# hhcho/sfgwas

Hardware: AMD Instinct MI355X
Metric: pca_power_iter_ring_macs_per_s (higher is better)
Workload: dtype u64 ring words, exact integers: int8 digits on the matrix core for the MAC of all five moduli, fp64-held integers in the encode and key-switch kernels

## Files before the change

sfgwas_amd/csrc/kernels.hpp:

```cpp
#pragma once
#include "common.hpp"
#include "mm_plan.hpp"
#include "assoc_plan.hpp"

constexpr int SFG_MAXPATTERN = 128;
struct ModPattern { int period; int8_t m[SFG_MAXPATTERN]; };
struct RowMap { int rpg; size_t gstride_in, gstride_out; };
struct PanelMap { int G, g, shift0; unsigned packed_mask = 0; int K = 0; };

int launch_ntt_fwd(sfg_ctx *ctx, const u64 *in, u64 *out, size_t nrows, const ModPattern &pat);
int launch_ntt_inv(sfg_ctx *ctx, const u64 *in, u64 *out, size_t nrows, const ModPattern &pat);
int launch_ntt_plain(sfg_ctx *ctx, const double *pc, u64 *out, size_t nplain, int L);
struct MoveJob;
struct PtRide;
int launch_ntt_plain_half(sfg_ctx *ctx, const double *pc, u64 *out_half, size_t nplain, int L, PanelMap pm, const uint32_t *perm = nullptr, const MoveJob *mv = nullptr);
int launch_expand_half(sfg_ctx *ctx, const u64 *half, u64 *full, size_t nrows);
int launch_ntt_fwd_map(sfg_ctx *ctx, const u64 *in, u64 *out, size_t nrows, const ModPattern &pat, const RowMap &rm);
int launch_ntt_inv_map(sfg_ctx *ctx, const u64 *in, u64 *out, size_t nrows, const ModPattern &pat, const RowMap &rm);
struct MacStrides { size_t rot_k, rot_r, pt_k, pt_n, out_n, out_r; bool pt_half = false; bool pt_packed = false; bool pt_digits = false; bool i8 = false; bool i8_big = false; bool pt_digits_big = false;
                    const int8_t *B_small = nullptr, *B_big = nullptr;
                    int pt_layout = 0, pt_L = 0;
                    int B_mode = 0;
                    const int8_t *A_small = nullptr, *A_big = nullptr; };
int launch_mac_i8_small(sfg_ctx *ctx, const double *rotf, size_t rotf_k_stride, size_t rotf_r_stride, int plane0, const u64 *pt, u64 *out, int K, int R, int r0, int Ncols,
                        int l0, int nl, int accumulate, const MacStrides &st);
int launch_mac_i8_big(sfg_ctx *ctx, const double *rotf, size_t rotf_k_stride, size_t rotf_r_stride, int plane0, const u64 *pt, u64 *out, int K, int R, int r0, int Ncols,
                      int l0, int accumulate, const MacStrides &st);
int launch_skew(sfg_ctx *ctx, const int8_t *blk, size_t ld, int r, int c, int transposed, int square, int8_t *D);
struct PcCache { double *slot = nullptr; int mode = 0; const uint32_t *perm = nullptr; };
int launch_encode_rows(sfg_ctx *ctx, const int8_t *D, int shift0, int nshift, int L, u64 *pt, bool half_rows = false, int G = 0, int g = 0, unsigned packed_mask = 0, const PcCache *pcache = nullptr,
                       PtRide *ride = nullptr);
int encode_rows_launches(const sfg_ctx *ctx, int nshift);
int i8_ride_prepare(sfg_ctx *ctx, const u64 *panel, int K, int Ncols, size_t pt_k, size_t pt_n, int layout, int L, int launches, PtRide &ride);
int i8_ride_finish(sfg_ctx *ctx, PtRide &ride);
int i8_ride_tiles(sfg_ctx *ctx, int K, int L, int8_t **Bs, int8_t **Bb);
struct I8Args;
void launch_i8_pack_pt_digits(hipStream_t q, const I8Args &a, unsigned items, bool big);
void launch_move_alone(hipStream_t q, const MoveJob &j);
int launch_share(sfg_ctx *ctx, const u64 *rows, size_t rows_ct_stride, const u64 *xr, size_t x_ct_stride, u64 *h, int nl, int nct);
int launch_add_rows(sfg_ctx *ctx, const u64 *a, size_t a_ct_stride, const u64 *b, size_t b_ct_stride, u64 *out, size_t out_ct_stride, int nl, int nct);
int encrypt_errors_moddown(sfg_ctx *ctx, const int32_t *e0, const int32_t *e1, int nct, int level, u64 *out);
int launch_geno_unpack(sfg_ctx *ctx, const sfg_geno *g, size_t r0, size_t c0, size_t nr, size_t nc, int8_t *out, size_t ld_out);
int launch_rotate_right(sfg_ctx *ctx, const u64 *in, u64 *out, int nct, int level, const int *nrot_host);
int launch_rotate_right_indexed(sfg_ctx *ctx, const u64 *in, int nin, u64 *out, int nct, int level, const int *nrot_host, const int *in_index);
int launch_rotate_right_indexed_f64(sfg_ctx *ctx, const u64 *in, int nin, double *outf, int nct, int level, const int *nrot_host, const int *in_index, int L,
                                    const size_t *out_slot = nullptr);
int launch_relinearize(sfg_ctx *ctx, const u64 *tmp, int nct, int level, const u64 *mid, u64 *out);
int launch_ct_add(sfg_ctx *ctx, const u64 *a, const u64 *b, u64 *out, size_t nct, int level);
int mac_dma_planes(sfg_ctx *ctx, int L, std::vector<int> &plane_of, std::vector<int> &is_big);
double mac_big_maxterm(u64 q);
int launch_rot_to_f64(sfg_ctx *ctx, const u64 *rot, size_t nrows, int nl_rot, int L, double *rotf);
int launch_mac_dma(sfg_ctx *ctx, const double *rotf, size_t rows_per_k, const u64 *pt, u64 *out, int K, int R, int Ncols, int L, int accumulate, const MacStrides &st,
                   const double *rotsum = nullptr);
int launch_rot_sum(sfg_ctx *ctx, const double *rotf, size_t rows_per_k, int K, int L, double *rotsum);
int launch_pack_pt(sfg_ctx *ctx, const u64 *in, u64 *out, size_t nrows, size_t words_per_row, int L, unsigned packed_mask);
unsigned mac_dma_packed_mask(sfg_ctx *ctx, int L);
bool mac_use_dma(const sfg_ctx *ctx);
int launch_mac_bc(sfg_ctx *ctx, const double *rotf, size_t rows_per_k, const u64 *pt, u64 *out, int K, int R, int Ncols, int L, int accumulate, const MacStrides &st,
                  const double *rotsum);
int rotcache_build_rows_tab(sfg_ctx *ctx, const u64 *A, int s, int in_level, int max_level, int nbr, int b0, int b1, const std::vector<std::vector<uint8_t>> *tabs, double *cache);
int assoc_build_rotcache(sfg_ctx *ctx, const u64 *A_dev, int s, int in_level, int max_level, size_t nr, const std::vector<size_t> &widths, double **out);
struct I8RotPre { int G = 0, nbr = 0, s = 0, L = 0; std::vector<int8_t *> As, Ab; };
int i8_rotpre_build(sfg_ctx *ctx, const u64 *A_dev, int s, int in_level, int max_level, int nbr, const std::vector<std::vector<uint8_t>> *tabs, size_t budget_bytes, const char *prefix, I8RotPre &pre);
void i8_rotpre_free(I8RotPre &pre);
int matmul_resident_range_i8pre(sfg_ctx *ctx, const I8RotPre &pre, int s, int max_level, const sfg_geno *g, unsigned flags, int blk0, int blk1, uint64_t *out);
int matmul_accumulate_i8pre(sfg_ctx *ctx, const I8RotPre &pre, int s, int max_level, const sfg_geno *g, unsigned flags, int j0, int j1, int accumulate, uint64_t *acc,
                            size_t acc_col_words = 0);
int launch_i8_pack_rot_to(sfg_ctx *ctx, const double *rotf, size_t rotf_k_stride, size_t rotf_r_stride, int plane0, int K, int R, int l0, int nl, bool big, int8_t *A_out);
struct AssocRot { double *f64 = nullptr; I8RotPre pre; };
int assoc_build_rot(sfg_ctx *ctx, const u64 *A_dev, int s, int in_level, int max_level, size_t nr, const std::vector<size_t> &widths, AssocRot &out);
void assoc_free_rot(AssocRot &r);
struct AssocRotScope { AssocRot r; ~AssocRotScope() { assoc_free_rot(r); } };
int assoc_product(sfg_ctx *ctx, const AssocRot &r, const uint64_t *A_dev, int s, int in_level, int max_level, const sfg_geno *g, unsigned flags, int nct, uint64_t *out);
int assoc_batch_tail(sfg_ctx *ctx, const u64 *tmp, const sfg_geno *g, int s, size_t nct, size_t ctw, uint64_t *out_dev, size_t out_ct_capacity, size_t out_shift,
                     double *sum_host, double *sqsum_host);

int launch_bed_decode(sfg_ctx *ctx, hipStream_t st, const uint8_t *dbed, size_t bps, size_t num_sample, size_t num_snp, const int32_t *rmap, const int32_t *cmap,
// ... 10 lines not shown
```

sfgwas_amd/csrc/matmul.hip:

```cpp
#include "common.hpp"
#include "kernels.hpp"
#include "i8_move.hpp"
#include <algorithm>
#include <string>

static inline int ceil_div(size_t a, size_t b) { return (int)((a + b - 1) / b); }

struct Shape {
    size_t nrow, ncol;
    int nbr, m_ct;
    bool transposed;
    const int8_t *dev; size_t ld;
    const sfg_geno *g;
    int rows_of(int bi) const { return (int)(std::min((size_t)(bi + 1) * SFG_SLOTS, nrow) - (size_t)bi * SFG_SLOTS); }
    int cols_of(int bj) const { return (int)(std::min((size_t)(bj + 1) * SFG_SLOTS, ncol) - (size_t)bj * SFG_SLOTS); }
    const int8_t *block(int bi, int bj) const {
        return transposed ? dev + (size_t)bj * SFG_SLOTS * ld + (size_t)bi * SFG_SLOTS
                          : dev + (size_t)bi * SFG_SLOTS * ld + (size_t)bj * SFG_SLOTS;
    }
};
static Shape make_shape(const sfg_geno *g, unsigned flags) {
    Shape sh; sh.transposed = (flags & SFG_TRANSPOSE) != 0;
    sh.nrow = sh.transposed ? g->ncol : g->nrow; sh.ncol = sh.transposed ? g->nrow : g->ncol;
    sh.nbr = ceil_div(sh.nrow, SFG_SLOTS); sh.m_ct = ceil_div(sh.ncol, SFG_SLOTS);
    sh.dev = g->dev; sh.ld = g->ld; sh.g = g; return sh;
}

__global__ void __launch_bounds__(256) k_drop_level(const u64 *in, u64 *out, int nl_in, int nl) {
    const int N = SFG_N; const size_t row = blockIdx.x / (N / 256);
    const size_t ctp = row / nl, m = row % nl;
    const size_t x = (blockIdx.x % (N / 256)) * 256 + threadIdx.x;
    out[row * N + x] = in[(ctp * nl_in + m) * N + x];
}
__global__ void __launch_bounds__(256) k_sum_giants(const u64 *rot, int ngiant, int s, int L, u64 *out, size_t out_i_stride,
                                                    int accumulate, const ModConst *modc) {
    const int N = SFG_N; const size_t row = blockIdx.x / (N / 256);
    const int i = (int)(row / (2 * L)), pl = (int)(row % (2 * L)), l = pl % L;
    const size_t x = (blockIdx.x % (N / 256)) * 256 + threadIdx.x;
    const double q = modc[l].q, qinv = modc[l].qinv;
    double acc = accumulate ? u64_to_f64(out[(size_t)i * out_i_stride + (size_t)pl * N + x]) : 0.0;
    for (int g = 0; g < ngiant; g++) {
        acc += u64_to_f64(rot[(((size_t)g * s + i) * 2 * L + pl) * N + x]);
        if ((g & 31) == 31) acc = pred(acc, q, qinv);
    }
    out[(size_t)i * out_i_stride + (size_t)pl * N + x] = f64_to_u64(canon(acc, q, qinv));
}
__global__ void __launch_bounds__(256) k_reduce_rows(u64 *rows, int L, const ModConst *modc) {
    const int N = SFG_N; const size_t row = blockIdx.x / (N / 256); const int l = (int)(row % L);
    const size_t off = row * N + (blockIdx.x % (N / 256)) * 256 + threadIdx.x;
    rows[off] = rows[off] % modc[l].qi;
}
__global__ void __launch_bounds__(256) k_pt_zero(u64 *pt, size_t pitch_words, size_t seg_words, int L, size_t prow, unsigned packed_mask) {
    const size_t seg = blockIdx.y, x = (size_t)blockIdx.x * 256 + threadIdx.x;
    if (x >= seg_words) return;
    const int l = (int)((x / prow) % L);
    pt[seg * pitch_words + x] = ((packed_mask >> l) & 1u) ? PACKED_ZERO : 0ULL;
}
__global__ void __launch_bounds__(256) k_pt_zero_kmajor(uint8_t *pt, int K, int planes, int n0, int k0, int nk) {
    const size_t blk = ((size_t)(n0 + blockIdx.y) * planes * 64 + blockIdx.x) * (size_t)K * 128 + (size_t)k0 * 128;
    uint4 *p = reinterpret_cast<uint4 *>(pt + blk);
    for (int i = threadIdx.x; i < nk * 8; i += 256) p[i] = make_uint4(0, 0, 0, 0);
}
static int launch_pt_zero_kmajor(sfg_ctx *ctx, u64 *pt, int K, int planes, int n0, int n1, int k0, int k1) {
    if (n1 <= n0 || k1 <= k0) return 0;
    hipLaunchKernelGGL(k_pt_zero_kmajor, dim3((unsigned)(planes * 64), (unsigned)(n1 - n0)), dim3(256), 0, ctx->stream, reinterpret_cast<uint8_t *>(pt), K, planes, n0, k0, k1 - k0);
    SFG_HIP(ctx, hipGetLastError());
    return 0;
}
static int launch_pt_zero(sfg_ctx *ctx, u64 *pt, size_t pitch_words, size_t seg_words, int nseg, int L, size_t prow, unsigned packed_mask) {
    if (!packed_mask) {
        if (nseg == 1) SFG_HIP(ctx, hipMemsetAsync(pt, 0, seg_words * 8, ctx->stream));
        else SFG_HIP(ctx, hipMemset2DAsync(pt, pitch_words * 8, 0, seg_words * 8, nseg, ctx->stream));
        return 0;
    }
    hipLaunchKernelGGL(k_pt_zero, dim3((unsigned)((seg_words + 255) / 256), (unsigned)nseg), dim3(256), 0, ctx->stream, pt, pitch_words, seg_words, L, prow, packed_mask);
    SFG_HIP(ctx, hipGetLastError());
    return 0;
}
// ... 452 lines not shown
                SFG_HIP(ctx, hipEventRecord(ctx->ev_pipe[(gi + 1) & 1], ctx->aux_stream));
            }
            SFG_HIP(ctx, hipStreamWaitEvent(main_stream, ctx->ev_pipe[gi & 1], 0));
            rotf_grp = c.rotf + (size_t)(gi & 1) * rot_half;
            if (c.rotsum) rotsum_grp = c.rotsum + (size_t)(gi & 1) * rotsum_half;
        } else SFG_TRY(build_group(c, bg, b1, 0));
        for (int bj = j0; bj < j1; bj++, it++) {
            pt = pt_base + (size_t)(plan.ride_want ? (it & 1) : 0) * plan.panel_words;
            PtRide ride;
            if (plan.ride_want && !c.rideBs) SFG_TRY(i8_ride_tiles(ctx, G * d, L, &c.rideBs, &c.rideBb));
            if (held.on && plan.ride_want && c.rideBs) {
                SFG_TRY(i8_ride_prepare(ctx, held.ptp, held.gsn * d, d, plan.plw, (size_t)held.gsn * d * plan.plw, plan.pt_layout, L, ride_launch_count(c, bg, ng, sh.cols_of(bj)), ride));
                if (ride.on && (ride.job.a5.B != c.rideBs || (ride.job.n6 && ride.job.a6.B != c.rideBb))) SFG_FAIL(ctx, "matmul: internal: the riding transposition's tile buffers moved");
            }
            if (held.on && !ride.on) { SFG_TRY(run_mac(c, held, c.rideBs ? 2 : 0)); held.on = false; }
            for (int g = 0; g < ng; g++) SFG_TRY(encode_block(c, bg + g, bj, g, ng, pt, ride.on ? &ride : nullptr));
            if (held.on) { SFG_TRY(i8_ride_finish(ctx, ride)); SFG_TRY(run_mac(c, held, 1)); held.on = false; }
            MacJob m; m.on = true; m.ptp = pt; m.gsn = ng; m.gi = gi;
            m.acc_flag = (accumulate || bg != b0) ? 1 : 0;
            m.accj = acc + (size_t)(bj - j0) * acc_col; m.rotf_grp = rotf_grp; m.rotsum_grp = rotsum_grp;
            if (plan.ride_want && c.rideBs) held = m;
            else SFG_TRY(run_mac(c, m, c.rideBs ? 2 : 0));
        }
    }
    if (held.on) rc = run_mac(c, held, 2);
    return rc;
}

static int matmul_finalize(sfg_ctx *ctx, const u64 *acc, int s, int max_level, int ncolb, int m_ct_out, int jout0, int g0, int g1,
                           const std::vector<uint8_t> *giant_active, int accumulate, u64 *out, int acc_giants = SFG_D, int giant_base = 0) {
    const int N = SFG_N, d = SFG_D, L = max_level;
    const size_t accw = (size_t)s * 2 * L * N, ctw = (size_t)2 * L * N;
    if (g0 < 0 || g1 > acc_giants || g0 > g1 || giant_base < 0) SFG_FAIL(ctx, "finalize: giant range out of bounds");
    u64 *rot = nullptr;
    SFG_TRY(sfg_scratch(ctx, "mm.fin_rot", (size_t)d * accw * 8, (void **)&rot));
    std::vector<int> glist;
    for (int g = g0; g < g1; g++) if (giant_base + g < d && (!giant_active || (*giant_active)[giant_base + g])) glist.push_back(g);
    const int ng = (int)glist.size();
    std::vector<int> nrv((size_t)ng * s), inv((size_t)ng * s);
    for (int k = 0; k < ng; k++) for (int i = 0; i < s; i++) { nrv[(size_t)k * s + i] = -(giant_base + glist[k]) * d; inv[(size_t)k * s + i] = glist[k] * s + i; }
    int rc = 0;
    for (int jb = 0; jb < ncolb && !rc; jb++) {
        const u64 *accj = acc + (size_t)jb * acc_giants * accw;
        u64 *o = out + (size_t)(jout0 + jb) * ctw;
        if (ng) {
            PhaseTimer t(ctx, "rotate");
            rc = launch_rotate_right_indexed(ctx, accj, acc_giants * s, rot, ng * s, L - 1, nrv.data(), inv.data());
            t.stop(1);
            if (rc) break;
        }
        hipLaunchKernelGGL(k_sum_giants, dim3((unsigned)((size_t)s * 2 * L * (N / 256))), dim3(256), 0, ctx->stream, rot, ng, s, L,
                           o, (size_t)m_ct_out * ctw, accumulate, ctx->modc);
        if (hipGetLastError() != hipSuccess) { rc = 1; ctx->err = "finalize: k_sum_giants launch failed"; }
    }
    return rc;
}

static void giant_table(const Shape &sh, std::vector<uint8_t> &giant_t) {
    giant_t.assign(SFG_D, 0);
    for (int bi = 0; bi < sh.nbr; bi++) {
        const int nr = sh.rows_of(bi);
        for (int shift = 0; shift < SFG_SLOTS; shift++) {
            if (giant_t[shift / SFG_D]) { shift = (shift / SFG_D + 1) * SFG_D - 1; continue; }
            bool any = false;
            for (int bj = 0; bj < sh.m_ct && !any; bj++) any = diag_bool(nr, sh.cols_of(bj), SFG_SLOTS, -shift);
            if (any) giant_t[shift / SFG_D] = 1;
        }
    }
}

extern "C" int sfg_matmul_accumulate_dev(sfg_ctx *ctx, const uint64_t *A, int s, int in_level, int max_level, const sfg_geno *g, unsigned flags,
                                         int b0, int b1, int j0, int j1, int accumulate, uint64_t *acc) {
    ApiScope api_scope(ctx);
    SFG_HIP(ctx, hipSetDevice(ctx->device));
    Shape sh = make_shape(g, flags);
    return matmul_accumulate(ctx, (const u64 *)A, s, in_level, max_level, sh, flags, b0, b1, j0, j1, accumulate, (u64 *)acc);
}
extern "C" int sfg_matmul_finalize_dev(sfg_ctx *ctx, const uint64_t *acc, int s, int max_level, int ncolb, int g0, int g1, int accumulate, uint64_t *out) {
    ApiScope api_scope(ctx);
    SFG_HIP(ctx, hipSetDevice(ctx->device));
    return matmul_finalize(ctx, (const u64 *)acc, s, max_level, ncolb, ncolb, 0, g0, g1, nullptr, accumulate, (u64 *)out);
}

extern "C" int sfg_matmul_finalize_slots_dev(sfg_ctx *ctx, const uint64_t *acc, int s, int max_level, int ncolb, int acc_giants, int giant_base,
                                             int g0, int g1, int accumulate, uint64_t *out) {
    ApiScope api_scope(ctx);
    SFG_HIP(ctx, hipSetDevice(ctx->device));
    if (acc_giants < 1) SFG_FAIL(ctx, "finalize: acc_giants must be positive");
// ... 515 lines not shown
```

sfgwas_amd/csrc/rotate.hip:

```cpp
#include "common.hpp"
#include "kernels.hpp"
#include "ksw.hpp"


static void fill_ext(const sfg_ctx *ctx, ExtConst &e, const std::vector<int> &src) {
    memset(&e, 0, sizeof e);
    e.a = (int)src.size();
    for (int m = 0; m < e.a; m++) e.src[m] = src[m];
    for (int m = 0; m < e.a; m++) {
        u64 qm = ctx->q[src[m]], h = 1;
        for (int k = 0; k < e.a; k++) if (k != m) h = h_mulmod(h, ctx->q[src[k]] % qm, qm);
        u64 hi = h_invmod(h, qm);
        e.qhat_inv[m] = (double)hi; e.qhat_inv_q[m] = (double)hi / (double)qm;
    }
    for (int t = 0; t < ctx->nmod; t++) {
        u64 qt = ctx->q[t], D = 1 % qt;
        for (int m = 0; m < e.a; m++) {
            u64 ht = 1 % qt;
            for (int k = 0; k < e.a; k++) if (k != m) ht = h_mulmod(ht, ctx->q[src[k]] % qt, qt);
            e.qhat_t[t][m] = (double)ht; e.qhat_t_q[t][m] = (double)ht / (double)qt;
            D = h_mulmod(D, ctx->q[src[m]] % qt, qt);
        }
        e.D_t[t] = (double)D; e.D_t_q[t] = (double)D / (double)qt;
    }
// ... 22 lines not shown
    }
    *host = kc;
    auto it = ctx->ksw_cache.find(level);
    if (it == ctx->ksw_cache.end()) {
        KswConst *d = nullptr;
        SFG_HIP(ctx, hipMalloc(&d, sizeof(KswConst)));
        SFG_HIP(ctx, hipMemcpy(d, &kc, sizeof(KswConst), hipMemcpyHostToDevice));
        ctx->ksw_cache[level] = d; *dev = d;
    } else *dev = (KswConst *)it->second;
    return 0;
}


__global__ void __launch_bounds__(256) k_ksw_extend(const u64 *c2, const u64 *ct_in, u64 *ext, const KswConst *kcp, const ModConst *modc) {
    const KswConst &kc = *kcp;
    const int N = SFG_N, x = blockIdx.x * 256 + threadIdx.x, i = blockIdx.y; const size_t b = blockIdx.z;
    const ExtConst &e = kc.dig[i];
    const u64 *c2b = c2 + b * (size_t)kc.nl * N;
    u64 *eb = ext + (b * kc.beta + i) * (size_t)kc.nt * N;
    double xs[KSW_MAXA], y[KSW_MAXA], v = 0.0;
#pragma unroll
    for (int m = 0; m < KSW_MAXA; m++) xs[m] = m < e.a ? u64_to_f64(c2b[(size_t)e.src[m] * N + x]) : 0.0;
    if (e.a > 1) ext_prepare(e, modc, xs, y, v);
    for (int t = 0; t < kc.nt; t++) {
        const int tg = kc.tmod[t];
        u64 outv;
        if (kc.digit_of[t] == i) continue;
        else if (e.a == 1) outv = f64_to_u64(canon(xs[0], modc[tg].q, modc[tg].qinv));
        else outv = f64_to_u64(ext_target(e, tg, modc[tg].q, modc[tg].qinv, y, v));
        eb[(size_t)t * N + x] = outv;
    }
}

__global__ void __launch_bounds__(256) k_ksw_inner(const u64 *ext, const u64 *ct_in, const u64 *const *keys, const int *inidx, u64 *acc, const KswConst *kcp, const ModConst *modc, int nmod) {
    const KswConst &kc = *kcp;
    const int N = SFG_N, x = 2 * (blockIdx.x * 256 + threadIdx.x), t = blockIdx.y; const size_t b = blockIdx.z;
    const int tg = kc.tmod[t];
    const double q = modc[tg].q, qinv = modc[tg].qinv;
    const u64 *key = keys[b];
    const size_t bi = (size_t)inidx[b];
    double a0x = 0.0, a0y = 0.0, a1x = 0.0, a1y = 0.0;
    for (int i = 0; i < kc.beta; i++) {
        const ulonglong2 ev = kc.digit_of[t] == i ? *reinterpret_cast<const ulonglong2 *>(ct_in + (bi * 2 * (size_t)kc.nl + kc.nl + t) * N + x)
                                                  : *reinterpret_cast<const ulonglong2 *>(ext + ((bi * kc.beta + i) * (size_t)kc.nt + t) * N + x);
        const ulonglong2 k0 = *reinterpret_cast<const ulonglong2 *>(key + (((size_t)i * 2 + 0) * nmod + tg) * N + x);
        const ulonglong2 k1 = *reinterpret_cast<const ulonglong2 *>(key + (((size_t)i * 2 + 1) * nmod + tg) * N + x);
        const double ex = u64_to_f64(ev.x), ey = u64_to_f64(ev.y);
        a0x += mulmod2(ex, u64_to_f64(k0.x), q, qinv); a0y += mulmod2(ey, u64_to_f64(k0.y), q, qinv);
        a1x += mulmod2(ex, u64_to_f64(k1.x), q, qinv); a1y += mulmod2(ey, u64_to_f64(k1.y), q, qinv);
    }
    *reinterpret_cast<ulonglong2 *>(acc + ((b * 2 + 0) * (size_t)kc.nt + t) * N + x) = make_ulonglong2(f64_to_u64(canon(a0x, q, qinv)), f64_to_u64(canon(a0y, q, qinv)));
    *reinterpret_cast<ulonglong2 *>(acc + ((b * 2 + 1) * (size_t)kc.nt + t) * N + x) = make_ulonglong2(f64_to_u64(canon(a1x, q, qinv)), f64_to_u64(canon(a1y, q, qinv)));
}

__global__ void __launch_bounds__(256) k_moddown_extend(const u64 *acc, u64 *ext2, const KswConst *kcp, const ModConst *modc) {
    const KswConst &kc = *kcp;
    const int N = SFG_N, x = blockIdx.x * 256 + threadIdx.x, p = blockIdx.y; const size_t b = blockIdx.z;
    const ExtConst &e = kc.pq;
    const u64 *ap = acc + ((b * 2 + p) * (size_t)kc.nt + kc.nl) * N;
    double xs[KSW_MAXA], y[KSW_MAXA], v = 0.0;
#pragma unroll
    for (int m = 0; m < KSW_MAXA; m++) xs[m] = m < e.a ? u64_to_f64(ap[(size_t)m * N + x]) : 0.0;
    if (e.a > 1) ext_prepare(e, modc, xs, y, v);
    for (int t = 0; t < kc.nl; t++) {
        u64 outv = e.a == 1 ? f64_to_u64(canon(xs[0], modc[t].q, modc[t].qinv)) : f64_to_u64(ext_target(e, t, modc[t].q, modc[t].qinv, y, v));
        ext2[((b * 2 + p) * (size_t)kc.nl + t) * N + x] = outv;
    }
}

struct F64Form { int on, L, centre; size_t rowf; int plane_of[SFG_MAXMOD], big[SFG_MAXMOD]; };
__device__ __forceinline__ void store_rot_f64(double *row, const F64Form &ff, int t, int x, double v, double q) {
    const int N = SFG_N;
    double *o = row + (size_t)ff.plane_of[t] * N;
    if (ff.big[t]) {
        const double wc = v > __builtin_floor(q * 0.5) ? v - q : v;
        const double hi = __builtin_floor((wc + 4194304.0) * 0x1p-23), lo = wc - hi * 8388608.0;
        o[2 * x] = lo; o[2 * x + 1] = hi;
    } else o[x] = (ff.centre && v > __builtin_floor(q * 0.5)) ? v - q : v;
}
__global__ void __launch_bounds__(256) k_ksw_finish(const u64 *ct_in, const int *inidx, const u64 *acc, const u64 *ext2, const uint16_t *const *index,
                                                   u64 *const *ct_out, const KswConst *kcp, const ModConst *modc, const u64 *add1, F64Form ff) {
    const KswConst &kc = *kcp;
    const int N = SFG_N, x = blockIdx.x * 256 + threadIdx.x, t = blockIdx.y; const size_t b = blockIdx.z;
    if (ff.on && t >= ff.L) return;
    const double q = modc[t].q, qinv = modc[t].qinv, pinv = kc.pinv[t], pinv_q = kc.pinv_q[t];
    const int src = index[b][x];
#pragma unroll
    for (int p = 0; p < 2; p++) {
        const double a = u64_to_f64(acc[((b * 2 + p) * (size_t)kc.nt + t) * N + src]);
        const double e = u64_to_f64(ext2[((b * 2 + p) * (size_t)kc.nl + t) * N + src]);
        double r = mulmod_lazy(a - e, pinv, pinv_q, q);
        if (p == 0) r += u64_to_f64(ct_in[((size_t)inidx[b] * 2 * (size_t)kc.nl + t) * N + src]);
        else if (add1) r += u64_to_f64(add1[((size_t)inidx[b] * (size_t)kc.nl + t) * N + src]);
        const double v = canon(r, q, qinv);
        if (ff.on) store_rot_f64(reinterpret_cast<double *>(ct_out[b]) + (size_t)p * ff.rowf, ff, t, x, v, q);
        else ct_out[b][((size_t)p * kc.nl + t) * N + x] = f64_to_u64(v);
    }
}

__global__ void __launch_bounds__(256) k_ct_add(const u64 *a, const u64 *b, u64 *out, int nl, const ModConst *modc, size_t total_rows) {
    const int N = SFG_N; const size_t row = blockIdx.x / (N / 256); const int m = (int)(row % nl);
    const u64 q = modc[m].qi;
    const size_t off = row * N + (blockIdx.x % (N / 256)) * 256 + threadIdx.x;
    u64 v = a[off] + b[off]; out[off] = v >= q ? v - q : v;
}

static int launch_keyswitch_jobs(sfg_ctx *ctx, const u64 *in, int nin, int level, const std::vector<int> &job_in, const std::vector<const u64 *> &keyp,
                                 const std::vector<const uint16_t *> &idxp, const std::vector<u64 *> &outp, const u64 *add1, const F64Form *ffp = nullptr) {
    const int N = SFG_N, nl = level + 1;
    F64Form ff; memset(&ff, 0, sizeof ff); if (ffp) ff = *ffp;
    KswConst *kcd; KswConst kc;
    SFG_TRY(get_ksw(ctx, level, &kcd, &kc));
    const size_t ctw = (size_t)2 * nl * N;
    const int nr = (int)job_in.size();
    if (!nr) return 0;
    const size_t in_rows = (size_t)nl + (size_t)kc.beta * kc.nt, job_rows = 2 * (size_t)kc.nt + 2 * (size_t)nl;
    const size_t budget = ctx->cfg.ksw_budget;
    int in_grp = (int)(budget / (in_rows * N * 8)); if (in_grp < 1) in_grp = 1; if (in_grp > nin) in_grp = nin;
    int chunk = (int)(budget / (job_rows * N * 8)); if (chunk < 1) chunk = 1; if (chunk > nr) chunk = nr;
    const size_t ptr_bytes = (size_t)nr * (3 * sizeof(void *) + sizeof(int)) + 256;
    const size_t ext_rows = (size_t)in_grp * kc.beta * kc.nt, ext2_rows = (size_t)chunk * 2 * nl;
    SFG_TRY(sfg_ws_reserve(ctx, (in_rows * in_grp + job_rows * chunk + ext_rows + ext2_rows) * N * 8 + ptr_bytes));
    u64 *c2 = (u64 *)ctx->ws, *ext = c2 + (size_t)in_grp * nl * N;
    u64 *acc = ext + ext_rows * N, *ext2 = acc + (size_t)chunk * 2 * kc.nt * N;
    u64 *extT = ext2 + ext2_rows * N, *ext2T = extT + ext_rows * N;
    const u64 **keys_all = (const u64 **)(ext2T + ext2_rows * N);
    const uint16_t **idx_all = (const uint16_t **)(keys_all + nr);
    u64 **out_all = (u64 **)(idx_all + nr);
    int *inidx_all = (int *)(out_all + nr);
    ModPattern pq; pq.period = nl; for (int m = 0; m < nl; m++) pq.m[m] = (int8_t)m;
    ModPattern pext; pext.period = kc.beta * kc.nt;
    for (int i = 0; i < kc.beta; i++) for (int t = 0; t < kc.nt; t++) pext.m[i * kc.nt + t] = kc.digit_of[t] == i ? (int8_t)-2 : (int8_t)kc.tmod[t];
    ModPattern pp; pp.period = kc.np; for (int p = 0; p < kc.np; p++) pp.m[p] = (int8_t)(ctx->nq + p);
    for (int i0 = 0; i0 < nin; i0 += in_grp) {
        const int ni = nin - i0 < in_grp ? nin - i0 : in_grp;
        std::vector<int> jobs;
        for (int k = 0; k < nr; k++) if (job_in[k] >= i0 && job_in[k] < i0 + ni) jobs.push_back(k);
        if (jobs.empty()) continue;
        const u64 *bin = in + (size_t)i0 * ctw;
        RowMap rm1; rm1.rpg = nl; rm1.gstride_in = ctw; rm1.gstride_out = (size_t)nl * N;
        SFG_TRY(launch_ntt_inv_map(ctx, bin + (size_t)nl * N, c2, (size_t)ni * nl, pq, rm1));
        hipLaunchKernelGGL(k_ksw_extend, dim3(N / 256, kc.beta, ni), dim3(256), 0, ctx->stream, c2, bin, ext, kcd, ctx->modc);
        SFG_HIP(ctx, hipGetLastError());
        SFG_TRY(launch_ntt_fwd(ctx, ext, extT, (size_t)ni * kc.beta * kc.nt, pext));
        {
            const size_t nj = jobs.size();
            std::vector<const u64 *> kp(nj); std::vector<const uint16_t *> ip(nj); std::vector<u64 *> op(nj); std::vector<int> ii(nj);
            for (size_t k = 0; k < nj; k++) { int jb = jobs[k]; kp[k] = keyp[jb]; ip[k] = idxp[jb]; op[k] = outp[jb]; ii[k] = job_in[jb] - i0; }
            SFG_TRY(sfg_upload_small(ctx, keys_all, kp.data(), nj * sizeof(void *)));
            SFG_TRY(sfg_upload_small(ctx, idx_all, ip.data(), nj * sizeof(void *)));
            SFG_TRY(sfg_upload_small(ctx, out_all, op.data(), nj * sizeof(void *)));
            SFG_TRY(sfg_upload_small(ctx, inidx_all, ii.data(), nj * sizeof(int)));
        }
        for (size_t c0 = 0; c0 < jobs.size(); c0 += chunk) {
            const int nb = (int)(jobs.size() - c0 < (size_t)chunk ? jobs.size() - c0 : (size_t)chunk);
            const u64 **keys_d = keys_all + c0; const uint16_t **idx_d = idx_all + c0; u64 **out_d = out_all + c0; int *inidx_d = inidx_all + c0;
            hipLaunchKernelGGL(k_ksw_inner, dim3(N / 512, kc.nt, nb), dim3(256), 0, ctx->stream, extT, bin, keys_d, inidx_d, acc, kcd, ctx->modc, ctx->nmod);
            SFG_HIP(ctx, hipGetLastError());
            RowMap rm4; rm4.rpg = kc.np; rm4.gstride_in = (size_t)kc.nt * N; rm4.gstride_out = (size_t)kc.nt * N;
            SFG_TRY(launch_ntt_inv_map(ctx, acc + (size_t)nl * N, acc + (size_t)nl * N, (size_t)nb * 2 * kc.np, pp, rm4));
            hipLaunchKernelGGL(k_moddown_extend, dim3(N / 256, 2, nb), dim3(256), 0, ctx->stream, acc, ext2, kcd, ctx->modc);
            SFG_HIP(ctx, hipGetLastError());
            SFG_TRY(launch_ntt_fwd(ctx, ext2, ext2T, (size_t)nb * 2 * nl, pq));
            hipLaunchKernelGGL(k_ksw_finish, dim3(N / 256, nl, nb), dim3(256), 0, ctx->stream, bin, inidx_d, acc, ext2T, idx_d, out_d, kcd, ctx->modc,
                               add1 ? add1 + (size_t)i0 * nl * N : nullptr, ff);
            SFG_HIP(ctx, hipGetLastError());
        }
    }
    return 0;
}
int launch_rotate_right_indexed(sfg_ctx *ctx, const u64 *in, int nin, u64 *out, int nct, int level, const int *nrot_host, const int *in_index) {
    const int N = SFG_N, nl = level + 1;
    if (level < 0 || level >= ctx->nq) SFG_FAIL(ctx, "rotate: level out of range");
    const size_t ctw = (size_t)2 * nl * N;
    std::vector<int> job_in; std::vector<const u64 *> keyp; std::vector<const uint16_t *> idxp; std::vector<u64 *> outp;
    for (int j = 0; j < nct; j++) {
        int nrot = nrot_host[j] % SFG_SLOTS; if (nrot < 0) nrot += SFG_SLOTS;
        const int src = in_index ? in_index[j] : j;
        if (src < 0 || src >= nin) SFG_FAIL(ctx, "rotate: input index out of range");
        if (nrot == 0) {
            int run = 1;
            while (j + run < nct && (nrot_host[j + run] % SFG_SLOTS) == 0 && (in_index ? in_index[j + run] : j + run) == src + run && src + run < nin) run++;
            SFG_HIP(ctx, hipMemcpyAsync(out + j * ctw, in + (size_t)src * ctw, (size_t)run * ctw * 8, hipMemcpyDeviceToDevice, ctx->stream));
            j += run - 1;
            continue;
        }
        u64 g = sfg_galois_for_rotation(ctx, SFG_SLOTS - nrot);
        auto it = ctx->rotkeys().find(g);
        if (it == ctx->rotkeys().end()) SFG_FAIL(ctx, "rotate: no rotation key loaded for right-rotation by %d (galois element %llu)", nrot, g);
        job_in.push_back(src); keyp.push_back(it->second.key_dev); idxp.push_back(it->second.index_dev); outp.push_back(out + j * ctw);
    }
    return launch_keyswitch_jobs(ctx, in, nin, level, job_in, keyp, idxp, outp, nullptr);
}
int launch_rotate_right_indexed_f64(sfg_ctx *ctx, const u64 *in, int nin, double *outf, int nct, int level, const int *nrot_host, const int *in_index, int L,
                                    const size_t *out_slot) {
    const int N = SFG_N, nl = level + 1;
    ctx->i8_gen++;
    if (level < 0 || level >= ctx->nq || L > nl) SFG_FAIL(ctx, "rotate: level out of range");
    const size_t ctw = (size_t)2 * nl * N;
    std::vector<int> plane_of, is_big; const int nplanes = mac_dma_planes(ctx, L, plane_of, is_big);
    if (nplanes < 0) return 1;
    F64Form ff; memset(&ff, 0, sizeof ff);
    ff.on = 1; ff.L = L; ff.centre = mac_dma_packed_mask(ctx, L) != 0; ff.rowf = (size_t)nplanes * N;
    for (int l = 0; l < L; l++) { ff.plane_of[l] = plane_of[l]; ff.big[l] = is_big[l]; }
    std::vector<int> job_in; std::vector<const u64 *> keyp; std::vector<const uint16_t *> idxp; std::vector<u64 *> outp;
    for (int j = 0; j < nct; j++) {
        int nrot = nrot_host[j] % SFG_SLOTS; if (nrot < 0) nrot += SFG_SLOTS;
        const int src = in_index ? in_index[j] : j;
        if (src < 0 || src >= nin) SFG_FAIL(ctx, "rotate: input index out of range");
        double *dst = outf + (out_slot ? out_slot[j] : (size_t)j) * 2 * ff.rowf;
        if (nrot == 0) {
            int run = 1;
            while (!out_slot && j + run < nct && (nrot_host[j + run] % SFG_SLOTS) == 0 && (in_index ? in_index[j + run] : j + run) == src + run && src + run < nin) run++;
            SFG_TRY(launch_rot_to_f64(ctx, in + (size_t)src * ctw, (size_t)2 * run, nl, L, dst));
            j += run - 1;
            continue;
        }
        u64 g = sfg_galois_for_rotation(ctx, SFG_SLOTS - nrot);
        auto it = ctx->rotkeys().find(g);
        if (it == ctx->rotkeys().end()) SFG_FAIL(ctx, "rotate: no rotation key loaded for right-rotation by %d (galois element %llu)", nrot, g);
        job_in.push_back(src); keyp.push_back(it->second.key_dev); idxp.push_back(it->second.index_dev); outp.push_back(reinterpret_cast<u64 *>(dst));
    }
    return launch_keyswitch_jobs(ctx, in, nin, level, job_in, keyp, idxp, outp, nullptr, &ff);
}
int launch_relinearize(sfg_ctx *ctx, const u64 *tmp, int nct, int level, const u64 *mid, u64 *out) {
// ... 49 lines not shown
```

Before: 6108 billion.

## Fuse giant-step rotations with summation in the key-switch tail

Replaces the finalize path, which rotated every giant-step ciphertext into scratch and then summed them, with a rotate-and-sum key switch. The automorphism is applied as a gather inside the inner key-switch product, so the per-job moddown and forward NTT are skipped. The moddown extension terms are accumulated per output in the coefficient domain, and a single forward NTT per output runs at the end. This removes the per-job NTTs and the full rotated-ciphertext buffers, at the cost of gathered loads, an added modulus-size restriction and more complex segment bookkeeping.

Measured after the change: 6120 billion, median of 2. No clear change (+0.2%).

```diff
diff --git a/sfgwas_amd/csrc/kernels.hpp b/sfgwas_amd/csrc/kernels.hpp
--- a/sfgwas_amd/csrc/kernels.hpp
+++ b/sfgwas_amd/csrc/kernels.hpp
@@ -43,6 +43,8 @@
 int launch_geno_unpack(sfg_ctx *ctx, const sfg_geno *g, size_t r0, size_t c0, size_t nr, size_t nc, int8_t *out, size_t ld_out);
 int launch_rotate_right(sfg_ctx *ctx, const u64 *in, u64 *out, int nct, int level, const int *nrot_host);
 int launch_rotate_right_indexed(sfg_ctx *ctx, const u64 *in, int nin, u64 *out, int nct, int level, const int *nrot_host, const int *in_index);
+int launch_rotate_sum_indexed(sfg_ctx *ctx, const u64 *in, int nin, int level, const int *nrot_host, const int *in_index, const int *out_index, int njobs, int nout,
+                              u64 *out, size_t out_stride, int accumulate);
 int launch_rotate_right_indexed_f64(sfg_ctx *ctx, const u64 *in, int nin, double *outf, int nct, int level, const int *nrot_host, const int *in_index, int L,
                                     const size_t *out_slot = nullptr);
 int launch_relinearize(sfg_ctx *ctx, const u64 *tmp, int nct, int level, const u64 *mid, u64 *out);
diff --git a/sfgwas_amd/csrc/matmul.hip b/sfgwas_amd/csrc/matmul.hip
--- a/sfgwas_amd/csrc/matmul.hip
+++ b/sfgwas_amd/csrc/matmul.hip
@@ -31,19 +31,6 @@
     const size_t ctp = row / nl, m = row % nl;
     const size_t x = (blockIdx.x % (N / 256)) * 256 + threadIdx.x;
     out[row * N + x] = in[(ctp * nl_in + m) * N + x];
-}
-__global__ void __launch_bounds__(256) k_sum_giants(const u64 *rot, int ngiant, int s, int L, u64 *out, size_t out_i_stride,
-                                                    int accumulate, const ModConst *modc) {
-    const int N = SFG_N; const size_t row = blockIdx.x / (N / 256);
-    const int i = (int)(row / (2 * L)), pl = (int)(row % (2 * L)), l = pl % L;
-    const size_t x = (blockIdx.x % (N / 256)) * 256 + threadIdx.x;
-    const double q = modc[l].q, qinv = modc[l].qinv;
-    double acc = accumulate ? u64_to_f64(out[(size_t)i * out_i_stride + (size_t)pl * N + x]) : 0.0;
-    for (int g = 0; g < ngiant; g++) {
-        acc += u64_to_f64(rot[(((size_t)g * s + i) * 2 * L + pl) * N + x]);
-        if ((g & 31) == 31) acc = pred(acc, q, qinv);
-    }
-    out[(size_t)i * out_i_stride + (size_t)pl * N + x] = f64_to_u64(canon(acc, q, qinv));
 }
 __global__ void __launch_bounds__(256) k_reduce_rows(u64 *rows, int L, const ModConst *modc) {
     const int N = SFG_N; const size_t row = blockIdx.x / (N / 256); const int l = (int)(row % L);
@@ -562,28 +549,20 @@
     const int N = SFG_N, d = SFG_D, L = max_level;
     const size_t accw = (size_t)s * 2 * L * N, ctw = (size_t)2 * L * N;
     if (g0 < 0 || g1 > acc_giants || g0 > g1 || giant_base < 0) SFG_FAIL(ctx, "finalize: giant range out of bounds");
-    u64 *rot = nullptr;
-    SFG_TRY(sfg_scratch(ctx, "mm.fin_rot", (size_t)d * accw * 8, (void **)&rot));
     std::vector<int> glist;
     for (int g = g0; g < g1; g++) if (giant_base + g < d && (!giant_active || (*giant_active)[giant_base + g])) glist.push_back(g);
     const int ng = (int)glist.size();
-    std::vector<int> nrv((size_t)ng * s), inv((size_t)ng * s);
-    for (int k = 0; k < ng; k++) for (int i = 0; i < s; i++) { nrv[(size_t)k * s + i] = -(giant_base + glist[k]) * d; inv[(size_t)k * s + i] = glist[k] * s + i; }
-    int rc = 0;
-    for (int jb = 0; jb < ncolb && !rc; jb++) {
+    std::vector<int> nrv((size_t)ng * s), inv((size_t)ng * s), outv((size_t)ng * s);
+    for (int k = 0; k < ng; k++) for (int i = 0; i < s; i++) { nrv[(size_t)k * s + i] = -(giant_base + glist[k]) * d; inv[(size_t)k * s + i] = glist[k] * s + i; outv[(size_t)k * s + i] = i; }
+    for (int jb = 0; jb < ncolb; jb++) {
         const u64 *accj = acc + (size_t)jb * acc_giants * accw;
-        u64 *o = out + (size_t)(jout0 + jb) * ctw;
-        if (ng) {
-            PhaseTimer t(ctx, "rotate");
-            rc = launch_rotate_right_indexed(ctx, accj, acc_giants * s, rot, ng * s, L - 1, nrv.data(), inv.data());
-            t.stop(1);
-            if (rc) break;
-        }
-        hipLaunchKernelGGL(k_sum_giants, dim3((unsigned)((size_t)s * 2 * L * (N / 256))), dim3(256), 0, ctx->stream, rot, ng, s, L,
-                           o, (size_t)m_ct_out * ctw, accumulate, ctx->modc);
-        if (hipGetLastError() != hipSuccess) { rc = 1; ctx->err = "finalize: k_sum_giants launch failed"; }
-    }
-    return rc;
+        PhaseTimer t(ctx, "rotate");
+        const int rc = launch_rotate_sum_indexed(ctx, accj, acc_giants * s, L - 1, nrv.data(), inv.data(), outv.data(), ng * s, s, out + (size_t)(jout0 + jb) * ctw,
+                                                 (size_t)m_ct_out * ctw, accumulate);
+        t.stop(1);
+        if (rc) return rc;
+    }
+    return 0;
 }
 
 static void giant_table(const Shape &sh, std::vector<uint8_t> &giant_t) {
diff --git a/sfgwas_amd/csrc/rotate.hip b/sfgwas_amd/csrc/rotate.hip
--- a/sfgwas_amd/csrc/rotate.hip
+++ b/sfgwas_amd/csrc/rotate.hip
@@ -78,19 +78,24 @@
     }
 }
 
-__global__ void __launch_bounds__(256) k_ksw_inner(const u64 *ext, const u64 *ct_in, const u64 *const *keys, const int *inidx, u64 *acc, const KswConst *kcp, const ModConst *modc, int nmod) {
+template <bool GATHER>
+__global__ void __launch_bounds__(256) k_ksw_inner(const u64 *ext, const u64 *ct_in, const u64 *const *keys, const int *inidx, const uint16_t *const *index, u64 *acc,
+                                                   const KswConst *kcp, const ModConst *modc, int nmod) {
     const KswConst &kc = *kcp;
     const int N = SFG_N, x = 2 * (blockIdx.x * 256 + threadIdx.x), t = blockIdx.y; const size_t b = blockIdx.z;
     const int tg = kc.tmod[t];
     const double q = modc[tg].q, qinv = modc[tg].qinv;
     const u64 *key = keys[b];
     const size_t bi = (size_t)inidx[b];
+    int sx = x, sy = x + 1;
+    if (GATHER) { const ushort2 sv = *reinterpret_cast<const ushort2 *>(index[b] + x); sx = sv.x; sy = sv.y; }
     double a0x = 0.0, a0y = 0.0, a1x = 0.0, a1y = 0.0;
     for (int i = 0; i < kc.beta; i++) {
-        const ulonglong2 ev = kc.digit_of[t] == i ? *reinterpret_cast<const ulonglong2 *>(ct_in + (bi * 2 * (size_t)kc.nl + kc.nl + t) * N + x)
-                                                  : *reinterpret_cast<const ulonglong2 *>(ext + ((bi * kc.beta + i) * (size_t)kc.nt + t) * N + x);
-        const ulonglong2 k0 = *reinterpret_cast<const ulonglong2 *>(key + (((size_t)i * 2 + 0) * nmod + tg) * N + x);
-        const ulonglong2 k1 = *reinterpret_cast<const ulonglong2 *>(key + (((size_t)i * 2 + 1) * nmod + tg) * N + x);
+        const u64 *er = kc.digit_of[t] == i ? ct_in + (bi * 2 * (size_t)kc.nl + kc.nl + t) * N : ext + ((bi * kc.beta + i) * (size_t)kc.nt + t) * N;
+        const u64 *k0r = key + (((size_t)i * 2 + 0) * nmod + tg) * N, *k1r = key + (((size_t)i * 2 + 1) * nmod + tg) * N;
+        ulonglong2 ev, k0, k1;
+        if (GATHER) { ev = make_ulonglong2(er[sx], er[sy]); k0 = make_ulonglong2(k0r[sx], k0r[sy]); k1 = make_ulonglong2(k1r[sx], k1r[sy]); }
+        else { ev = *reinterpret_cast<const ulonglong2 *>(er + x); k0 = *reinterpret_cast<const ulonglong2 *>(k0r + x); k1 = *reinterpret_cast<const ulonglong2 *>(k1r + x); }
         const double ex = u64_to_f64(ev.x), ey = u64_to_f64(ev.y);
         a0x += mulmod2(ex, u64_to_f64(k0.x), q, qinv); a0y += mulmod2(ey, u64_to_f64(k0.y), q, qinv);
         a1x += mulmod2(ex, u64_to_f64(k1.x), q, qinv); a1y += mulmod2(ey, u64_to_f64(k1.y), q, qinv);
@@ -144,6 +149,74 @@
     }
 }
 
+constexpr int KSW_SUM_MAXNL = SFG_MAXMOD - 1;
+constexpr u64 KSW_SUM_QMAX = 1ULL << 47;
+struct SumTail {
+    int nout = 0;
+    std::vector<int> job_out, ginv, copy_in, copy_out;
+    u64 *S = nullptr, *E = nullptr, *ET = nullptr;
+};
+__global__ void __launch_bounds__(256) k_ksw_sum_tail(const u64 *ct_in, const u64 *acc, const int *seg_off, const int *seg_out, const int *tj, int c0, const int *inidx,
+                                                     const uint16_t *const *index, const int *ginv, u64 *S, u64 *E, const KswConst *kcp, const ModConst *modc) {
+    const KswConst &kc = *kcp;
+    const int N = SFG_N, x = blockIdx.x * 256 + threadIdx.x, p = blockIdx.y, sg = blockIdx.z, nl = kc.nl;
+    const ExtConst &pq = kc.pq;
+    const size_t orow = ((size_t)seg_out[sg] * 2 + p) * nl;
+    double s[KSW_SUM_MAXNL], e[KSW_SUM_MAXNL];
+#pragma unroll
+    for (int t = 0; t < KSW_SUM_MAXNL; t++) if (t < nl) { s[t] = u64_to_f64(S[(orow + t) * N + x]); e[t] = u64_to_f64(E[(orow + t) * N + x]); }
+    int n = 0;
+    for (int k = seg_off[sg]; k < seg_off[sg + 1]; k++, n++) {
+        const int pos = tj[k];
+        const u64 *ab = acc + ((size_t)(pos - c0) * 2 + p) * (size_t)kc.nt * N;
+        const bool neg = (((unsigned)x * (unsigned)ginv[pos]) & (2u * N - 1)) >= (unsigned)N;
+        double xs[KSW_MAXA], y[KSW_MAXA], v = 0.0;
+#pragma unroll
+        for (int m = 0; m < KSW_MAXA; m++) {
+            xs[m] = 0.0;
+            if (m < pq.a) { const double r = u64_to_f64(ab[(size_t)(nl + m) * N + x]); xs[m] = (neg && r != 0.0) ? modc[pq.src[m]].q - r : r; }
+        }
+        if (pq.a > 1) ext_prepare(pq, modc, xs, y, v);
+        const u64 *c0r = ct_in + (size_t)inidx[pos] * 2 * nl * N + (p == 0 ? index[pos][x] : 0);
+#pragma unroll
+        for (int t = 0; t < KSW_SUM_MAXNL; t++) if (t < nl) {
+            const double q = modc[t].q, qinv = modc[t].qinv;
+            const double ev = pq.a == 1 ? canon(xs[0], q, qinv) : ext_target(pq, t, q, qinv, y, v);
+            e[t] += neg ? -ev : ev;
+            s[t] += mulmod_lazy(u64_to_f64(ab[(size_t)t * N + x]), kc.pinv[t], kc.pinv_q[t], q);
+            if (p == 0) s[t] += u64_to_f64(c0r[(size_t)t * N]);
+        }
+        if ((n & 15) == 15) {
+#pragma unroll
+            for (int t = 0; t < KSW_SUM_MAXNL; t++) if (t < nl) { s[t] = pred(s[t], modc[t].q, modc[t].qinv); e[t] = pred(e[t], modc[t].q, modc[t].qinv); }
+        }
+    }
+#pragma unroll
+    for (int t = 0; t < KSW_SUM_MAXNL; t++) if (t < nl) {
+        const double q = modc[t].q, qinv = modc[t].qinv;
+        S[(orow + t) * N + x] = f64_to_u64(canon(pred(s[t], q, qinv), q, qinv));
+        E[(orow + t) * N + x] = f64_to_u64(canon(pred(e[t], q, qinv), q, qinv));
+    }
+}
+__global__ void __launch_bounds__(256) k_ksw_sum_copy(const u64 *in, const int *cin, const int *cout, u64 *S, int nl, const ModConst *modc) {
+    const int N = SFG_N, x = blockIdx.x * 256 + threadIdx.x, row = blockIdx.y; const size_t c = blockIdx.z;
+    const u64 q = modc[row % nl].qi;
+    u64 *o = S + ((size_t)cout[c] * 2 * nl + row) * N + x;
+    const u64 v = *o + in[((size_t)cin[c] * 2 * nl + row) * N + x];
+    *o = v >= q ? v - q : v;
+}
+__global__ void __launch_bounds__(256) k_ksw_sum_finish(const u64 *S, const u64 *ET, u64 *out, size_t out_stride, int accumulate, const KswConst *kcp, const ModConst *modc) {
+    const KswConst &kc = *kcp;
+    const int N = SFG_N, x = blockIdx.x * 256 + threadIdx.x, row = blockIdx.y, t = row % kc.nl; const size_t o = blockIdx.z;
+    const double q = modc[t].q, qinv = modc[t].qinv;
+    const size_t w = (o * 2 * kc.nl + row) * N + x;
+    double r = u64_to_f64(S[w]);
+    if (ET) r -= mulmod_lazy(u64_to_f64(ET[w]), kc.pinv[t], kc.pinv_q[t], q);
+    u64 *dst = out + o * out_stride + (size_t)row * N + x;
+    if (accumulate) r += u64_to_f64(*dst);
+    *dst = f64_to_u64(canon(r, q, qinv));
+}
+
 __global__ void __launch_bounds__(256) k_ct_add(const u64 *a, const u64 *b, u64 *out, int nl, const ModConst *modc, size_t total_rows) {
     const int N = SFG_N; const size_t row = blockIdx.x / (N / 256); const int m = (int)(row % nl);
     const u64 q = modc[m].qi;
@@ -152,28 +225,49 @@
 }
 
 static int launch_keyswitch_jobs(sfg_ctx *ctx, const u64 *in, int nin, int level, const std::vector<int> &job_in, const std::vector<const u64 *> &keyp,
-                                 const std::vector<const uint16_t *> &idxp, const std::vector<u64 *> &outp, const u64 *add1, const F64Form *ffp = nullptr) {
+                                 const std::vector<const uint16_t *> &idxp, const std::vector<u64 *> &outp, const u64 *add1, const F64Form *ffp = nullptr,
+                                 SumTail *sum = nullptr) {
     const int N = SFG_N, nl = level + 1;
     F64Form ff; memset(&ff, 0, sizeof ff); if (ffp) ff = *ffp;
     KswConst *kcd; KswConst kc;
     SFG_TRY(get_ksw(ctx, level, &kcd, &kc));
     const size_t ctw = (size_t)2 * nl * N;
     const int nr = (int)job_in.size();
-    if (!nr) return 0;
-    const size_t in_rows = (size_t)nl + (size_t)kc.beta * kc.nt, job_rows = 2 * (size_t)kc.nt + 2 * (size_t)nl;
+    if (!nr && !sum) return 0;
+    if (sum && nl > KSW_SUM_MAXNL) SFG_FAIL(ctx, "rotate-and-sum: level %d unsupported (more than %d moduli)", level, KSW_SUM_MAXNL);
+    if (sum) for (int t = 0; t < nl; t++) if (ctx->q[t] >= KSW_SUM_QMAX) SFG_FAIL(ctx, "rotate-and-sum: modulus %d is not below 2^47 (the lazy sums of 16 jobs would pass 2^53)", t);
+    const size_t in_rows = (size_t)nl + (size_t)kc.beta * kc.nt, job_rows = 2 * (size_t)kc.nt + (sum ? 0 : 2 * (size_t)nl);
     const size_t budget = ctx->cfg.ksw_budget;
-    int in_grp = (int)(budget / (in_rows * N * 8)); if (in_grp < 1) in_grp = 1; if (in_grp > nin) in_grp = nin;
+    int in_grp = (int)(budget / (in_rows * N * 8)); if (in_grp < 1) in_grp = 1; if (in_grp > nin) in_grp = nin; if (!nr) in_grp = 0;
     int chunk = (int)(budget / (job_rows * N * 8)); if (chunk < 1) chunk = 1; if (chunk > nr) chunk = nr;
-    const size_t ptr_bytes = (size_t)nr * (3 * sizeof(void *) + sizeof(int)) + 256;
-    const size_t ext_rows = (size_t)in_grp * kc.beta * kc.nt, ext2_rows = (size_t)chunk * 2 * nl;
-    SFG_TRY(sfg_ws_reserve(ctx, (in_rows * in_grp + job_rows * chunk + ext_rows + ext2_rows) * N * 8 + ptr_bytes));
-    u64 *c2 = (u64 *)ctx->ws, *ext = c2 + (size_t)in_grp * nl * N;
+    const size_t ncopy = sum ? sum->copy_in.size() : 0;
+    const size_t ptr_bytes = (size_t)nr * (3 * sizeof(void *) + sizeof(int)) + 256
+                           + (sum ? ((size_t)nr * 4 + 2 * ncopy + 4) * sizeof(int) : 0);
+    const size_t sum_rows = sum ? (size_t)sum->nout * 2 * nl : 0;
+    const size_t ext_rows = (size_t)in_grp * kc.beta * kc.nt, ext2_rows = sum ? 0 : (size_t)chunk * 2 * nl;
+    SFG_TRY(sfg_ws_reserve(ctx, (3 * sum_rows + in_rows * in_grp + job_rows * chunk + ext_rows + ext2_rows) * N * 8 + ptr_bytes));
+    u64 *c2 = (u64 *)ctx->ws + 3 * sum_rows * N, *ext = c2 + (size_t)in_grp * nl * N;
     u64 *acc = ext + ext_rows * N, *ext2 = acc + (size_t)chunk * 2 * kc.nt * N;
     u64 *extT = ext2 + ext2_rows * N, *ext2T = extT + ext_rows * N;
     const u64 **keys_all = (const u64 **)(ext2T + ext2_rows * N);
     const uint16_t **idx_all = (const uint16_t **)(keys_all + nr);
     u64 **out_all = (u64 **)(idx_all + nr);
     int *inidx_all = (int *)(out_all + nr);
+    int *ginv_all = inidx_all + nr, *tj_all = ginv_all + nr, *segoff_all = tj_all + nr, *segout_all = segoff_all + nr + 1, *copy_all = segout_all + nr + 1;
+    if (sum) {
+        sum->S = (u64 *)ctx->ws; sum->E = sum->S + sum_rows * N; sum->ET = sum->E + sum_rows * N;
+        SFG_HIP(ctx, hipMemsetAsync(sum->S, 0, 2 * sum_rows * N * 8, ctx->stream));
+        std::vector<char> done(ncopy, 0);
+        for (size_t left = ncopy; left;) {
+            std::vector<int> ci, co; std::set<int> seen;
+            for (size_t c = 0; c < ncopy; c++) if (!done[c] && seen.insert(sum->copy_out[c]).second) { ci.push_back(sum->copy_in[c]); co.push_back(sum->copy_out[c]); done[c] = 1; left--; }
+            SFG_TRY(sfg_upload_small(ctx, copy_all, ci.data(), ci.size() * sizeof(int)));
+            SFG_TRY(sfg_upload_small(ctx, copy_all + ncopy, co.data(), co.size() * sizeof(int)));
+            hipLaunchKernelGGL(k_ksw_sum_copy, dim3(N / 256, 2 * nl, (unsigned)ci.size()), dim3(256), 0, ctx->stream, in, copy_all, copy_all + ncopy, sum->S, nl, ctx->modc);
+            SFG_HIP(ctx, hipGetLastError());
+        }
+        if (!nr) return 0;
+    }
     ModPattern pq; pq.period = nl; for (int m = 0; m < nl; m++) pq.m[m] = (int8_t)m;
     ModPattern pext; pext.period = kc.beta * kc.nt;
     for (int i = 0; i < kc.beta; i++) for (int t = 0; t < kc.nt; t++) pext.m[i * kc.nt + t] = kc.digit_of[t] == i ? (int8_t)-2 : (int8_t)kc.tmod[t];
@@ -198,13 +292,38 @@
             SFG_TRY(sfg_upload_small(ctx, out_all, op.data(), nj * sizeof(void *)));
             SFG_TRY(sfg_upload_small(ctx, inidx_all, ii.data(), nj * sizeof(int)));
         }
+        std::vector<int> seg_first(1, 0);
+        if (sum) {
+            const size_t nj = jobs.size();
+            std::vector<int> gi(nj), tj(nj), soff, sout;
+            for (size_t k = 0; k < nj; k++) { gi[k] = sum->ginv[jobs[k]]; tj[k] = (int)k; }
+            for (size_t c0 = 0; c0 < nj; c0 += chunk) {
+                const size_t c1 = std::min(nj, c0 + (size_t)chunk);
+                std::stable_sort(tj.begin() + c0, tj.begin() + c1, [&](int a, int b) { return sum->job_out[jobs[a]] < sum->job_out[jobs[b]]; });
+                for (size_t k = c0; k < c1; k++) if (k == c0 || sum->job_out[jobs[tj[k]]] != sout.back()) { soff.push_back((int)k); sout.push_back(sum->job_out[jobs[tj[k]]]); }
+                seg_first.push_back((int)soff.size());
+            }
+            soff.push_back((int)nj);
+            SFG_TRY(sfg_upload_small(ctx, ginv_all, gi.data(), nj * sizeof(int)));
+            SFG_TRY(sfg_upload_small(ctx, tj_all, tj.data(), nj * sizeof(int)));
+            SFG_TRY(sfg_upload_small(ctx, segoff_all, soff.data(), soff.size() * sizeof(int)));
+            SFG_TRY(sfg_upload_small(ctx, segout_all, sout.data(), sout.size() * sizeof(int)));
+        }
         for (size_t c0 = 0; c0 < jobs.size(); c0 += chunk) {
             const int nb = (int)(jobs.size() - c0 < (size_t)chunk ? jobs.size() - c0 : (size_t)chunk);
             const u64 **keys_d = keys_all + c0; const uint16_t **idx_d = idx_all + c0; u64 **out_d = out_all + c0; int *inidx_d = inidx_all + c0;
-            hipLaunchKernelGGL(k_ksw_inner, dim3(N / 512, kc.nt, nb), dim3(256), 0, ctx->stream, extT, bin, keys_d, inidx_d, acc, kcd, ctx->modc, ctx->nmod);
+            if (sum) hipLaunchKernelGGL(k_ksw_inner<true>, dim3(N / 512, kc.nt, nb), dim3(256), 0, ctx->stream, extT, bin, keys_d, inidx_d, idx_d, acc, kcd, ctx->modc, ctx->nmod);
+            else hipLaunchKernelGGL(k_ksw_inner<false>, dim3(N / 512, kc.nt, nb), dim3(256), 0, ctx->stream, extT, bin, keys_d, inidx_d, idx_d, acc, kcd, ctx->modc, ctx->nmod);
             SFG_HIP(ctx, hipGetLastError());
             RowMap rm4; rm4.rpg = kc.np; rm4.gstride_in = (size_t)kc.nt * N; rm4.gstride_out = (size_t)kc.nt * N;
             SFG_TRY(launch_ntt_inv_map(ctx, acc + (size_t)nl * N, acc + (size_t)nl * N, (size_t)nb * 2 * kc.np, pp, rm4));
+            if (sum) {
+                const int ci = (int)(c0 / chunk), nseg = seg_first[ci + 1] - seg_first[ci];
+                hipLaunchKernelGGL(k_ksw_sum_tail, dim3(N / 256, 2, nseg), dim3(256), 0, ctx->stream, bin, acc, segoff_all + seg_first[ci], segout_all + seg_first[ci], tj_all,
+                                   (int)c0, inidx_all, idx_all, ginv_all, sum->S, sum->E, kcd, ctx->modc);
+                SFG_HIP(ctx, hipGetLastError());
+                continue;
+            }
             hipLaunchKernelGGL(k_moddown_extend, dim3(N / 256, 2, nb), dim3(256), 0, ctx->stream, acc, ext2, kcd, ctx->modc);
             SFG_HIP(ctx, hipGetLastError());
             SFG_TRY(launch_ntt_fwd(ctx, ext2, ext2T, (size_t)nb * 2 * nl, pq));
@@ -237,6 +356,38 @@
         job_in.push_back(src); keyp.push_back(it->second.key_dev); idxp.push_back(it->second.index_dev); outp.push_back(out + j * ctw);
     }
     return launch_keyswitch_jobs(ctx, in, nin, level, job_in, keyp, idxp, outp, nullptr);
+}
+int launch_rotate_sum_indexed(sfg_ctx *ctx, const u64 *in, int nin, int level, const int *nrot_host, const int *in_index, const int *out_index, int njobs, int nout,
+                              u64 *out, size_t out_stride, int accumulate) {
+    const int N = SFG_N, nl = level + 1;
+    if (level < 0 || level >= ctx->nq) SFG_FAIL(ctx, "rotate: level out of range");
+    if (nout <= 0) return 0;
+    SumTail sum; sum.nout = nout;
+    std::vector<int> job_in; std::vector<const u64 *> keyp; std::vector<const uint16_t *> idxp;
+    for (int j = 0; j < njobs; j++) {
+        int nrot = nrot_host[j] % SFG_SLOTS; if (nrot < 0) nrot += SFG_SLOTS;
+        const int src = in_index ? in_index[j] : j;
+        if (src < 0 || src >= nin) SFG_FAIL(ctx, "rotate: input index out of range");
+        if (out_index[j] < 0 || out_index[j] >= nout) SFG_FAIL(ctx, "rotate: output index out of range");
+        if (nrot == 0) { sum.copy_in.push_back(src); sum.copy_out.push_back(out_index[j]); continue; }
+        const u64 g = sfg_galois_for_rotation(ctx, SFG_SLOTS - nrot);
+        auto it = ctx->rotkeys().find(g);
+        if (it == ctx->rotkeys().end()) SFG_FAIL(ctx, "rotate: no rotation key loaded for right-rotation by %d (galois element %llu)", nrot, g);
+        u64 gi = g; for (int k = 0; k < 5; k++) gi = gi * (2 - g * gi);
+        job_in.push_back(src); keyp.push_back(it->second.key_dev); idxp.push_back(it->second.index_dev);
+        sum.job_out.push_back(out_index[j]); sum.ginv.push_back((int)(gi & (2ULL * N - 1)));
+    }
+    std::vector<u64 *> outp(job_in.size(), nullptr);
+    SFG_TRY(launch_keyswitch_jobs(ctx, in, nin, level, job_in, keyp, idxp, outp, nullptr, nullptr, &sum));
+    KswConst *kcd; KswConst kc;
+    SFG_TRY(get_ksw(ctx, level, &kcd, &kc));
+    if (!job_in.empty()) {
+        ModPattern pq; pq.period = nl; for (int m = 0; m < nl; m++) pq.m[m] = (int8_t)m;
+        SFG_TRY(launch_ntt_fwd(ctx, sum.E, sum.ET, (size_t)nout * 2 * nl, pq));
+    }
+    hipLaunchKernelGGL(k_ksw_sum_finish, dim3(N / 256, 2 * nl, nout), dim3(256), 0, ctx->stream, sum.S, job_in.empty() ? nullptr : sum.ET, out, out_stride, accumulate, kcd, ctx->modc);
+    SFG_HIP(ctx, hipGetLastError());
+    return 0;
 }
 int launch_rotate_right_indexed_f64(sfg_ctx *ctx, const u64 *in, int nin, double *outf, int nct, int level, const int *nrot_host, const int *in_index, int L,
                                     const size_t *out_slot) {
```
